# lukasc-ch/CBinfer

Measured on AMD Instinct MI355X. Metric: frames/sec + effective GFLOP/s vs dense, scene-labeling CNN 480x320 @10% change, higher is better.
Workload: dtype f32-equivalent: f32 tensors, every operand as three bf16 terms (24 bits, exact), six products on the bf16 MFMA, f32 accumulate; 1 GPU; sceneLabeling CBConv2d coarse-grained fp32, synthetic 480x320 seq @10% change (32x32 re-drawn blocks), experiment 6, one sequence per GPU; sequences_per_gpu=1, launch=program

## Files before the change

### cbinfer_amd/csrc/cb_split.hip

```cpp
#include <stdlib.h>

#include <type_traits>

#include "cb_common.h"

#ifdef CBS_STAMP
__device__ unsigned long long cbs_stamp_buf[4 * 2048 * 16];
#define CB_TAIL_STAMP(i)                                                                 \
    do {                                                                                 \
        if (threadIdx.x == 0 && blockIdx.x < 2048)                                       \
            cbs_stamp_buf[(2 * 2048 + blockIdx.x) * 16 + (i)] = __builtin_amdgcn_s_memrealtime(); \
    } while (0)
#define CBS_DET_STAMP(i)                                                                                            \
    do {                                                                                                            \
        const unsigned wg = blockIdx.y * gridDim.x + blockIdx.x;                                                    \
        if (POOL && threadIdx.x == 0 && blockIdx.z == 0 && wg < 2048)                                               \
            cbs_stamp_buf[(3 * 2048 + wg) * 16 + (i)] = __builtin_amdgcn_s_memrealtime();                            \
    } while (0)
#else
#define CBS_DET_STAMP(i)
#endif
#include "cb_tail_core.h"
#include "cb_split_common.h"

// ... 1468 lines not shown
                    }
                }
                __syncthreads();
#pragma unroll 1
                for (int c = 0; c < nNext; ++c) {
                    const CbhNext& nx = ext.L[q].next[c];
                    if (t < BN && ((s_nchg[c * (BN / 32) + (t >> 5)] >> (t & 31)) & 1u)) {
                        const int pix = s_tilePix[t];
                        const int py = cbs_div(pix, p.magicW), px = pix - py * p.W;
                        cbh_or_dilated(nx.masks, py, px, p.H, p.W, p.wpr, nx.kHH, nx.kWH);
                    }
                }
            }
        }
        CBS_STAMP_AT(5);
#ifdef CBS_STAMP
        cbs_first = false;
#endif
    }

    if constexpr (SIDE) {
        if (ext.sideFrame) {
            const int busy = min(items, (int)gridDim.x), nIdle = (int)gridDim.x - busy;
            const bool idleDo = nIdle >= 32;
            const int parts = idleDo ? nIdle : (int)gridDim.x, part = idleDo ? (int)blockIdx.x - busy : (int)blockIdx.x;
            if (part >= 0) {
                const int per = (ext.sideHW + parts - 1) / parts;
                const int i1 = min(ext.sideHW, (part + 1) * per);
                for (int i = part * per + t; i < i1; i += NT) {
                    bool chg = false;
                    for (int c = 0; c < ext.sideC; ++c)
                        chg |= cb_changed(ext.sideState[(long)c * ext.sideHW + i], ext.sideFrame[(long)c * ext.sideHW + i],
                                          ext.sideTh);
                    if (chg)
                        for (int c = 0; c < ext.sideC; ++c)
                            ext.sideState[(long)c * ext.sideHW + i] = ext.sideFrame[(long)c * ext.sideHW + i];
                }
            }
        }
    }

    if (totAll == 0) return;
    __syncthreads();
    if (t == 0) {
        int* ctl = (int*)(p.seq[0].masks + 2 * (long)MW);
        const int nSh = p.arriveShards;
        int last = 0;
        if (nSh <= 1) {
            last = __hip_atomic_fetch_add(ctl + 2, 1, __ATOMIC_RELAXED, __HIP_MEMORY_SCOPE_AGENT) == (int)gridDim.x - 1;
        } else {
            const int sh = blockIdx.x % nSh, expected = ((int)gridDim.x - sh + nSh - 1) / nSh;
            int* c = (int*)(p.seq[0].masks + (long)MW) + sh * 32;
            if (__hip_atomic_fetch_add(c, 1, __ATOMIC_RELAXED, __HIP_MEMORY_SCOPE_AGENT) == expected - 1) {
                __hip_atomic_store(c, 0, __ATOMIC_RELAXED, __HIP_MEMORY_SCOPE_AGENT);
                const int active = min(nSh, (int)gridDim.x);
                last = __hip_atomic_fetch_add(ctl + 2, 1, __ATOMIC_RELAXED, __HIP_MEMORY_SCOPE_AGENT) == active - 1;
            }
        }
        s_wsum[0] = last;
    }
    __syncthreads();
    if (s_wsum[0]) {
        for (int i = t; i < E; i += NT) {
            const int q = cbs_div(i, p.magicMW), w = i - q * MW;
            ((unsigned long long*)s_maskPtr[q])[w] = 0ull;
        }
        if (t == 0) {
            int* ctl = (int*)(p.seq[0].masks + 2 * (long)MW);
            __hip_atomic_store(ctl + 2, 0, __ATOMIC_RELAXED, __HIP_MEMORY_SCOPE_AGENT);
        }
    }
}

#define CBS_TILES_BEFORE(tilesBefore, info) \
    int tilesBefore[CBS_MAXSEQ + 1];        \
    tilesBefore[0] = 0;                     \
    _Pragma("unroll") for (int q_ = 0; q_ < CBS_MAXSEQ; ++q_) tilesBefore[q_ + 1] = tilesBefore[q_] + (info)[CBS_INFO_TP + q_]
#define CBS_TILE_SEQUENCE(q, tilesBefore, nSeq, ptg)  \
    int q = 0;                                        \
    _Pragma("unroll") for (int u_ = 1; u_ < CBS_MAXSEQ; ++u_) if (u_ < (nSeq) && (ptg) >= tilesBefore[u_]) q = u_

__global__ __launch_bounds__(256) void cbs_reduce_kernel(CbsParams p, int BM, int BN) {
    cb_touch_kernarg<sizeof(CbsParams) + 8>();
    const int SK = p.info[CBS_INFO_SK];
    if (SK <= 1) return;
    const int MT = p.info[CBS_INFO_MT], CMB = MT * SK, TILE4 = BM * BN / 4, HW = p.H * p.W;
    CBS_TILES_BEFORE(tilesBefore, p.info);
    const int TP = tilesBefore[CBS_MAXSEQ];
    const float4* __restrict__ slabs = (const float4*)p.slabs;
    const long total = (long)TP * MT * TILE4;
    for (long g = (long)blockIdx.x * 256 + threadIdx.x; g < total; g += (long)gridDim.x * 256) {
        const int tile = (int)(g / TILE4), c = (int)(g - (long)tile * TILE4);
        const int ptg = tile / MT, mt = tile % MT;
        const int nl = c % BN, mq = c / BN;
        CBS_TILE_SEQUENCE(q, tilesBefore, p.nSeq, ptg);
        const int n = (ptg - tilesBefore[q]) * BN + nl;
        const int N = p.info[CBS_INFO_TP + CBS_MAXSEQ + q];
        const float4* sl = slabs + ((long)ptg * CMB + mt) * TILE4 + c;
        const int pix = n < N ? p.seq[q].listOut[n] : -1;
        float s0 = 0.f, s1 = 0.f, s2 = 0.f, s3 = 0.f;
        for (int j0 = 0; j0 < SK; j0 += 8) {
            float4 v[8];
#pragma unroll
            for (int j = 0; j < 8; ++j)
                if (j0 + j < SK) v[j] = sl[(long)(j0 + j) * MT * TILE4];
#pragma unroll
            for (int j = 0; j < 8; ++j)
                if (j0 + j < SK) s0 += v[j].x, s1 += v[j].y, s2 += v[j].z, s3 += v[j].w;
        }
        if ((unsigned)pix >= (unsigned)HW) continue;
        const int m = mt * BM + 4 * mq;
        const float sv[4] = {s0, s1, s2, s3};
        float* out = p.seq[q].out;
#pragma unroll
        for (int e = 0; e < 4; ++e) {
            if (m + e >= p.K) continue;
            const float bv = !p.bias ? 0.f : (p.halfOut ? (float)((const _Float16*)p.bias)[m + e] : p.bias[m + e]);
            float v = fmaf(sv[e], p.outScale, bv);
            if (p.relu) v = v <= 0.f ? 0.f : v;
            if (p.halfOut) {
                ((_Float16*)out)[(long)(m + e) * HW + pix] = (_Float16)v;
                continue;
            }
            if (p.accumulate) {
                v += out[(long)(m + e) * HW + pix];
                float* rp = p.seq[q].reluOut;
                if (rp) rp[(long)(m + e) * HW + pix] = v <= 0.f ? 0.f : v;
            }
            out[(long)(m + e) * HW + pix] = v;
        }
    }
}

template <int BM, int BN>
__global__ __launch_bounds__(256) void cbh_reduce_kernel(CbsParams p, CbhExt ext) {
    cb_touch_kernarg<sizeof(CbsParams) + sizeof(CbhExt)>();
    if (p.info[CBS_INFO_SK] <= 1) return;
    const int MT = p.info[CBS_INFO_MT], TILE4 = BM * BN / 4, HW = p.H * p.W;
    int tilesBefore[CBH_GROUP + 1], slabBase[CBH_GROUP], chQ[CBH_GROUP];
    tilesBefore[0] = 0;
    {
        int run = 0;
#pragma unroll
        for (int q = 0; q < CBH_GROUP; ++q) {
            const int tq = p.info[CBS_INFO_TP + q];
            chQ[q] = p.info[CBS_INFO_CH + q];
            tilesBefore[q + 1] = tilesBefore[q] + tq;
            slabBase[q] = run;
            run += tq * MT * chQ[q];
        }
    }
    constexpr int PXG = 16, GP = BN / PXG;
    const int groups = tilesBefore[CBH_GROUP] * GP;
    const int t = threadIdx.x, px = t & 15;
    __shared__ unsigned s_chg[CBH_NEXT];
    const float4* __restrict__ slabs = (const float4*)p.slabs;
    const int QT = MT * (BM / 4);
    const int NCC = (QT + 31) / 32;
    for (int unit = blockIdx.x; unit < groups * NCC; unit += gridDim.x) {
        const int g = unit / NCC, cc = unit - g * NCC;
        const int ptg = g / GP, gi = g - ptg * GP;
        int q = 0;
#pragma unroll
        for (int u = 1; u < CBH_GROUP; ++u)
            if (u < p.nSeq && ptg >= tilesBefore[u]) q = u;
        const int n0 = (ptg - tilesBefore[q]) * BN + gi * PXG;
        const int N = p.info[CBS_INFO_TP + CBS_MAXSEQ + q];
        if (n0 >= N) continue;
        static_assert(CBH_GROUP == 2, "two layers");
        const int SK = q ? chQ[1] : chQ[0], CMB = MT * SK;
        const long tileSlab = (q ? slabBase[1] : slabBase[0]) + (long)(ptg - tilesBefore[q]) * CMB;
        const CbhLayer& L = ext.L[q];
        const int Kq = L.K, nNext = L.nNext;
        int pix = n0 + px < N ? p.seq[q].listOut[n0 + px] : -1;
        if ((unsigned)pix >= (unsigned)HW) pix = -1;
        const int pixLd = max(pix, 0);
        const int py = cbs_div(pixLd, p.magicW), pxx = pixLd - py * p.W;
        __syncthreads();
        if (t < CBH_NEXT) s_chg[t] = 0u;
        __syncthreads();
        _Float16* out = (_Float16*)p.seq[q].out;
        bool chg[CBH_NEXT];
#pragma unroll
        for (int c = 0; c < CBH_NEXT; ++c) chg[c] = false;
        const float4* sl0 = slabs + tileSlab * TILE4 + gi * PXG + px;
        const int nx2 = nNext > 1 ? 1 : 0;
        {
            const int cq0 = cc * 32 + (t >> 4);
            float4 v[2][8];
            _Float16 s4[2][CBH_NEXT][4];
            float acc[2][4];
#pragma unroll
            for (int u = 0; u < 2; ++u) {
                const int cq = min(cq0 + 16 * u, QT - 1);
                const int mt = cq / (BM / 4), mq = cq - mt * (BM / 4), m = mt * BM + 4 * mq;
                const float4* sl = sl0 + (long)mt * TILE4 + mq * BN;
#pragma unroll
                for (int j = 0; j < 8; ++j) v[u][j] = sl[(long)min(j, SK - 1) * MT * TILE4];
#pragma unroll
                for (int e = 0; e < 4; ++e) {
                    const long o = (long)min(m + e, Kq - 1) * HW + pixLd;
                    s4[u][0][e] = nNext > 0 ? L.next[0].state[o] : (_Float16)0;
                    if (CBH_NEXT > 1) s4[u][CBH_NEXT > 1 ? 1 : 0][e] = nNext > 0 ? L.next[nx2].state[o] : (_Float16)0;
                }
            }
#pragma unroll
            for (int u = 0; u < 2; ++u) {
                float s0 = 0.f, s1 = 0.f, s2 = 0.f, s3 = 0.f;
#pragma unroll
                for (int j = 0; j < 8; ++j)
                    if (j < SK) s0 += v[u][j].x, s1 += v[u][j].y, s2 += v[u][j].z, s3 += v[u][j].w;
                acc[u][0] = s0, acc[u][1] = s1, acc[u][2] = s2, acc[u][3] = s3;
            }
            if (SK > 8) {
#pragma unroll
                for (int u = 0; u < 2; ++u) {
                    const int cq = min(cq0 + 16 * u, QT - 1);
                    const int mt = cq / (BM / 4), mq = cq - mt * (BM / 4);
                    const float4* sl = sl0 + (long)mt * TILE4 + mq * BN;
#pragma unroll
                    for (int j = 0; j < 8; ++j) v[u][j] = sl[(long)min(8 + j, SK - 1) * MT * TILE4];
                }
#pragma unroll
                for (int u = 0; u < 2; ++u)
#pragma unroll
                    for (int j = 0; j < 8; ++j)
                        if (8 + j < SK)
                            acc[u][0] += v[u][j].x, acc[u][1] += v[u][j].y, acc[u][2] += v[u][j].z, acc[u][3] += v[u][j].w;
            }
#pragma unroll
            for (int u = 0; u < 2; ++u) {
                const int cq = cq0 + 16 * u;
                if (cq >= QT) continue;
                const int mt = cq / (BM / 4), mq = cq - mt * (BM / 4), m = mt * BM + 4 * mq;
                if (pix < 0 || m >= Kq) continue;
                _Float16 hv[4];
#pragma unroll
                for (int e = 0; e < 4; ++e) {
                    const float bv = (L.bias && m + e < Kq) ? (float)L.bias[m + e] : 0.f;
                    float r = fmaf(acc[u][e], p.outScale, bv);
                    if (L.relu) r = r <= 0.f ? 0.f : r;
                    hv[e] = m + e < Kq ? (_Float16)r : (_Float16)0;
                    if (m + e < Kq) out[(long)(m + e) * HW + pix] = hv[e];
                }
#pragma unroll
                for (int c = 0; c < CBH_NEXT; ++c) {
                    if (c >= nNext) continue;
                    const CbhNext& nx = L.next[c];
                    _Float16* nst = nx.state;
                    const _Float16 thc = (_Float16)nx.th;
                    unsigned dm = 0u;
                    bool ch = false;
#pragma unroll
                    for (int e = 0; e < 4; ++e) {
                        if (m + e >= Kq) continue;
                        ch |= cb_changed(s4[u][c][e], hv[e], thc);
                        dm |= (unsigned)cb_differs(s4[u][c][e], hv[e]) << e;
                    }
                    chg[c] |= ch;
                    if (dm) {
#pragma unroll
                        for (int e = 0; e < 4; ++e)
                            if ((dm >> e) & 1u) nst[(long)(m + e) * HW + pix] = hv[e];
                        if (m < (nx.rec >> 1)) {
                            typedef _Float16 halfx4 __attribute__((ext_vector_type(4)));
                            char* rec = nx.S + CBS_SPAD + ((long)(py + nx.padY) * nx.Wp + (pxx + nx.padXL)) * nx.rec;
                            *(halfx4*)(rec + m * 2) = halfx4{hv[0], hv[1], hv[2], hv[3]};
                        }
                    }
                }
            }
        }
        if (nNext > 0) {
#pragma unroll
            for (int c = 0; c < CBH_NEXT; ++c)
                if (c < nNext && chg[c]) atomicOr(&s_chg[c], 1u << px);
            __syncthreads();
            for (int c = 0; c < nNext; ++c) {
                const CbhNext& nx = L.next[c];
                const int dy = (t >> 4) - nx.kHH, yy = py + dy;
                if (pix >= 0 && ((s_chg[c] >> px) & 1u) && dy <= nx.kHH && yy >= 0 && yy < p.H)
                    cbh_or_dilated(nx.masks, yy, pxx, p.H, p.W, p.wpr, 0, nx.kWH);
            }
        }
    }
}

struct CbsTailArgs {
    const float* w1p;
    const float* b1;
    const float* w2;
    const float* b2;
    float* out[CBS_MAXSEQ];
    int C1, C2, relu1, relu2;
};
template <int BM, int BN, int S>
__global__ __launch_bounds__(S == 1 ? 64 * CB_TAIL_MAXW : CB_TAIL_MAXT) void cbs_reduce_tail_kernel(CbsParams p,
                                                                                                  CbsTailArgs ta) {
    extern __shared__ __attribute__((aligned(16))) float cbs_tail_sm[];
    cb_touch_kernarg<sizeof(CbsParams) + sizeof(CbsTailArgs)>();
    const int C0 = p.K, C0P = (C0 + 15) / 16 * 16, C1 = ta.C1, C2 = ta.C2, HW = p.H * p.W;
    const int t = threadIdx.x, NT = blockDim.x;
    CB_TAIL_STAMP(0);
    const int SK = p.info[CBS_INFO_SK], MT = p.info[CBS_INFO_MT], CMB = MT * SK, TILE4 = BM * BN / 4;
    CBS_TILES_BEFORE(tilesBefore, p.info);
    const int GP = BN / CB_TAIL_PX, groups = tilesBefore[CBS_MAXSEQ] * GP;
    if ((int)blockIdx.x >= groups) return;
    CB_TAIL_STAMP(1);
    const CbTailLds L = cb_tail_lds(cbs_tail_sm, C0P, C1, C2);
    __shared__ int s_pix[CB_TAIL_PX];
    for (int i = t; i < C2 * C1; i += NT) L.W2s[i] = ta.w2[i];
    for (int i = t; i < C2; i += NT) L.b2s[i] = ta.b2[i];
    const float4* __restrict__ slabs = (const float4*)p.slabs;
    const bool hasBias = p.bias != nullptr;
    const float* biasp = hasBias ? p.bias : ta.b1;
    const int px = t & 15, cstep = NT >> 4;
    for (int g = blockIdx.x; g < groups; g += gridDim.x) {
        const int ptg = g / GP, gi = g - ptg * GP;
        CBS_TILE_SEQUENCE(q, tilesBefore, p.nSeq, ptg);
        const int nl0 = gi * CB_TAIL_PX, n0 = (ptg - tilesBefore[q]) * BN + nl0;
        const int N = p.info[CBS_INFO_TP + CBS_MAXSEQ + q];
        if (n0 >= N) continue;
        float* outq = p.seq[q].out;
        float* relq = p.accumulate ? p.seq[q].reluOut : nullptr;
        int pixMine = -1;
        if (n0 + px < N) pixMine = p.seq[q].listOut[n0 + px];
        int tq = t >> 4;
        asm volatile("" : "+v"(tq));
        if ((unsigned)pixMine >= (unsigned)HW) pixMine = -1;
        const int pixLd = max(pixMine, 0);
        if (SK > 1) {
            const float4* sl0 = slabs + (long)ptg * CMB * TILE4 + nl0 + px;
            const int QN = C0P / 4, perThread = (QN + cstep - 1) / cstep;
            auto slabRounds = [&](auto uc) {
                constexpr int U = decltype(uc)::value;
                const int rounds = (QN + U * cstep - 1) / (U * cstep);
                for (int rd = 0; rd < rounds; ++rd) {
                    const int cq0 = tq + rd * U * cstep;
                    float4 v[U][CBS_CHUNKS], bq[U];
#pragma unroll
                    for (int u = 0; u < U; ++u) {
                        const int cq = min(cq0 + u * cstep, QN - 1), mt = cq / (BM / 4), mq = cq - mt * (BM / 4);
#pragma unroll
                        for (int j = 0; j < CBS_CHUNKS; ++j) v[u][j] = sl0[((long)j * MT + mt) * TILE4 + mq * BN];
                        bq[u] = *(const float4*)(biasp + (hasBias ? min(4 * cq, p.K - 4) : 0));
                    }
                    __builtin_amdgcn_sched_barrier(0);
                    if (rd == 0) {
                        __syncthreads();
                        if (t < CB_TAIL_PX) s_pix[t] = pixMine;
                        CB_TAIL_STAMP(2);
                    }
#pragma unroll
                    for (int u = 0; u < U; ++u) {
                        const int cq = cq0 + u * cstep;
                        float s0 = 0.f, s1 = 0.f, s2 = 0.f, s3 = 0.f;
#pragma unroll
                        for (int j = 0; j < CBS_CHUNKS; ++j)
                            s0 += v[u][j].x, s1 += v[u][j].y, s2 += v[u][j].z, s3 += v[u][j].w;
                        const float sv[4] = {s0, s1, s2, s3}, bv[4] = {bq[u].x, bq[u].y, bq[u].z, bq[u].w};
#pragma unroll
                        for (int e = 0; e < 4; ++e) {
                            const int m = 4 * cq + e;
                            float r = fmaf(sv[e], p.outScale, hasBias ? bv[e] : 0.f);
                            if (p.relu) r = r <= 0.f ? 0.f : r;
                            if (cq < QN) {
                                if (p.accumulate) {
                                    if (pixMine >= 0 && m < p.K) {
                                        r += outq[(long)m * HW + pixMine];
                                        outq[(long)m * HW + pixMine] = r;
                                        if (relq) {
                                            r = r <= 0.f ? 0.f : r;
                                            relq[(long)m * HW + pixMine] = r;
                                        }
                                    }
                                } else if (pixMine >= 0 && m < p.K) {
                                    outq[(long)m * HW + pixMine] = r;
                                }
                                L.Xs[m * CB_TAIL_PX + px] = (m < p.K && pixMine >= 0) ? r : 0.f;
                            }
                        }
                    }
                }
            };
            if (perThread <= 1) slabRounds(std::integral_constant<int, 1>());
            else if (perThread <= 2 || S > 1) slabRounds(std::integral_constant<int, 2>());
            else slabRounds(std::integral_constant<int, 4>());
        } else {
            __syncthreads();
            if (t < CB_TAIL_PX) s_pix[t] = pixMine;
            const float* gsrc = relq ? relq : outq;
            cb_tail_gather<(S == 1 ? 16 : 8)>(L.Xs, gsrc, HW, pixLd, pixMine >= 0, C0, C0P, tq, px, cstep);
        }
        asm volatile("" ::: "memory");
        CbTailPre<S> P;
        cb_tail_preload<S>(P, ta.w1p, ta.b1, C0P, C1);
        CB_TAIL_STAMP(3);
        cb_tail_tile<S>(L, s_pix, P, ta.w1p, ta.out[q], C0P, C1, C2, HW, ta.relu1, ta.relu2);
        CB_TAIL_STAMP(7);
    }
}

template <int BM, int BN, int WM, int WN, int PRE_CAP, bool MASK_LDS, int RING, int AR = 0>
int cbs_launch_conv(const CbsParams& p, int perCU, const CbsTailArgs* tail, hipStream_t s,
                    const typename CbsExtOf<AR>::type& ext = typename CbsExtOf<AR>::type()) {
    if ((long)p.nSeq * p.maskWords > PRE_CAP) return CB_ERR_UNSUPPORTED;
    const bool second = p.slabs && (p.nStages >= 48 || p.forceSK > 0);
    if (tail && !second) return CB_ERR_UNSUPPORTED;
    dim3 grid((unsigned)(perCU * cb_num_cus())), block(64 * WM * WN);
    hipLaunchKernelGGL((cbs_conv_kernel<BM, BN, WM, WN, PRE_CAP, MASK_LDS, RING, AR>), grid, block, 0, s, p, ext);
    int st = cb_launch_status();
    if (st != CB_OK) return st;
    if constexpr (AR == 1) {
        if (second) {
            hipLaunchKernelGGL((cbh_reduce_kernel<BM, BN>), dim3(2 * cb_num_cus()), dim3(256), 0, s, p, ext);
            st = cb_launch_status();
        }
        return st;
    }
    if (tail) {
        const int S = cb_tail_chain_sets(p.K, tail->C1);
        auto* k = S == 4 ? cbs_reduce_tail_kernel<BM, BN, 4> : S == 2 ? cbs_reduce_tail_kernel<BM, BN, 2>
                                                                      : cbs_reduce_tail_kernel<BM, BN, 1>;
        const int waves = (tail->C1 + 15) / 16 * S, perCU = waves > 8 ? 1 : 2;
        hipLaunchKernelGGL(k, dim3(perCU * cb_num_cus()), dim3(64 * waves), cb_tail_lds_bytes(p.K, tail->C1, tail->C2), s, p,
                           *tail);
        st = cb_launch_status();
    } else if (second) {
        hipLaunchKernelGGL(cbs_reduce_kernel, dim3(4 * cb_num_cus()), dim3(256), 0, s, p, BM, BN);
        st = cb_launch_status();
    }
    return st;
}

}
using namespace cbs;

#ifdef CBS_STAMP
extern "C" int cbinfer_debug_split_stamps(void* host, long bytes, int clear) {
    if (clear) {
        void* d = nullptr;
        if (hipGetSymbolAddress(&d, HIP_SYMBOL(cbs_stamp_buf)) != hipSuccess) return -1;
        return (int)hipMemset(d, 0, sizeof(unsigned long long) * 4 * 2048 * 16);
    }
    return (int)hipMemcpyFromSymbol(host, HIP_SYMBOL(cbs_stamp_buf), (size_t)bytes);
}
#endif

template <typename Ext>
static int cbs_fill_side(Ext& e, const cbSideRefresh* side) {
    CB_REQUIRE(side->state && side->C >= 1 && side->H >= 1 && side->W >= 1 && (long)side->H * side->W < (1l << 30));
    e.sideFrame = side->frame, e.sideState = side->state, e.sideC = side->C, e.sideHW = side->H * side->W;
    e.sideTh = side->threshold;
    return CB_OK;
}

extern "C" {

int cbinfer_split_supported(int C, int K, int kH, int kW) { return cbs_supported(C, K, kH, kW) ? 1 : 0; }
int cbinfer_split_max_sequences(void) { return CBS_MAXSEQ; }
long cbinfer_split_max_mask_words(int K) { return cbs_bm(K) >= 128 ? CBS_PRE_BIG : CBS_PRE_MID; }

long cbinfer_split_state_bytes(int C, int H, int W, int kH, int kW) {
    const CbsGeom g = cbs_geom(C, H, W, kH, kW);
    return CBS_SPAD + (long)g.Hp * g.Wp * g.rec;
}
long cbinfer_split3_state_bytes(int C, int H, int W, int kH, int kW) {
    const CbsGeom g = cbs_geom(C, H, W, kH, kW, 3);
    return CBS_SPAD + (long)g.Hp * g.Wp * g.rec;
}

static long cbs_plain_offset(long aBytes, int nStages) { return (aBytes + (long)nStages * 4 + 15) / 16 * 16; }
long cbinfer_split_prepared_bytes(int C, int K, int kH, int kW) {
    const CbsGeom g = cbs_geom(C, 64, 64, kH, kW);
    return cbs_plain_offset((long)g.nStages * (cbs_kp(K) / 32) * 4096, g.nStages) + (long)K * C * kH * kW * 4;
}
long cbinfer_split3_prepared_bytes(int C, int K, int kH, int kW) {
    const CbsGeom g = cbs_geom(C, 64, 64, kH, kW, 3);
    return cbs_plain_offset((long)g.nStages * (cbs_kp(K) / 32) * 6144, g.nStages);
}

static long cbs_slab_capacity(int nSeq, int H, int W, int K) {
    const int bm = cbs_bm(K), bn = bm >= 128 ? 128 : 64;
    const long tiles = (long)nSeq * (((long)H * W + bn - 1) / bn) * (cbs_kp(K) / bm);
    return tiles > 2l * cb_num_cus() ? tiles : 2l * cb_num_cus();
}
static long cbs_workspace_bytes(int nSeq, int H, int W, int K) {
    const int bm = cbs_bm(K), bn = bm >= 128 ? 128 : 64;
    return 256 + cbs_slab_capacity(nSeq, H, W, K) * bm * bn * 4;
}
long cbinfer_split_workspace_bytes(int nSeq, int C, int H, int W, int K, int kH, int kW) {
    if (!cbs_supported(C, K, kH, kW)) return 0;
    if (cbs_geom(C, H, W, kH, kW).nStages < 48) return 0;
    return cbs_workspace_bytes(nSeq, H, W, K);
}

static void cbs_fill_params(CbsParams& p, const CbsGeom& g, int K, int KP, int BM, int H, int W, long MW, void* workspace,
                            long cap) {
    p.info = workspace ? (int*)workspace : nullptr;
    p.slabs = workspace ? (float*)((char*)workspace + 256) : nullptr;
    p.K = K, p.KP = KP, p.H = H, p.W = W, p.Wp = g.Wp, p.rec = g.rec, p.nStages = g.nStages, p.kH = g.kH, p.kW = g.kW;
    p.maskWords = (int)MW, p.wpr = cbinfer_mask_words_per_row(W), p.dummyBase = g.dummyBase;
    p.stateBytes = (long)g.Hp * g.Wp * g.rec;
    p.magicMW = (1ull << 32) / (unsigned long long)MW + 1ull;
    p.magicWpr = (1ull << 32) / (unsigned long long)p.wpr + 1ull;
    p.magicW = (1ull << 32) / (unsigned long long)W + 1ull;
    p.magicMT = (1ull << 32) / (unsigned long long)(KP / BM) + 1ull;
    p.arriveShards = (int)(MW / 16 < 8 ? MW / 16 : 8);
    p.slabCap = (int)(cap > 0x7fffffffl ? 0x7fffffffl : cap);
    p.splitRounds = 2;
    p.dbg = 0;
}

static int cbs_prep_weights(const float* weight, void* prepared, int K, int C, int kH, int kW, int H, int W, int planes,
                            float weightScale, cbStream_t stream) {
    if (!cbs_supported(C, K, kH, kW)) return CB_ERR_UNSUPPORTED;
    const CbsGeom g = cbs_geom(C, H, W, kH, kW, planes);
    if ((long)g.Hp * g.Wp * g.rec >= (1l << 31)) return CB_ERR_UNSUPPORTED;
    const int KP = cbs_kp(K);
    const long total = (long)g.nStages * (KP / 32) * (2 * planes) * 64;
    const long aBytes = total * 16;
    int* stageOff = (int*)((char*)prepared + aBytes);
    float* wPlain = planes == 3 ? nullptr : (float*)((char*)prepared + cbs_plain_offset(aBytes, g.nStages));
    hipLaunchKernelGGL(cbs_prep_kernel, dim3(cb_div_up(total > g.nStages ? total : g.nStages, 256)), dim3(256), 0,
                       (hipStream_t)stream, weight, (halfx8*)prepared, stageOff, wPlain, g, K, KP, weightScale);
    return cb_launch_status();
}
int cbinfer_split_prep_weights(const float* weight, void* prepared, int K, int C, int kH, int kW, int H, int W,
                               float weightScale, cbStream_t stream) {
    CB_REQUIRE(weight && prepared && H > 0 && W > 0 && weightScale > 0.f);
    return cbs_prep_weights(weight, prepared, K, C, kH, kW, H, W, 2, weightScale, stream);
}
int cbinfer_split3_prep_weights(const float* weight, void* prepared, int K, int C, int kH, int kW, int H, int W,
                                cbStream_t stream) {
    CB_REQUIRE(weight && prepared && H > 0 && W > 0);
    return cbs_prep_weights(weight, prepared, K, C, kH, kW, H, W, 3, 1.0f, stream);
}

static int cbs_state_init(void* splitState, int C, int H, int W, int kH, int kW, int planes, cbStream_t stream) {
    CB_REQUIRE(splitState && H > 0 && W > 0);
    if (!cbs_supported(C, 1, kH, kW)) return CB_ERR_UNSUPPORTED;
    const CbsGeom g = cbs_geom(C, H, W, kH, kW, planes);
    hipLaunchKernelGGL(cbs_state_init_kernel, dim3(1024), dim3(256), 0, (hipStream_t)stream, (uint4*)splitState, g);
    return cb_launch_status();
}
int cbinfer_split_state_init(void* splitState, int C, int H, int W, int kH, int kW, cbStream_t stream) {
    return cbs_state_init(splitState, C, H, W, kH, kW, 2, stream);
}
int cbinfer_split3_state_init(void* splitState, int C, int H, int W, int kH, int kW, cbStream_t stream) {
    return cbs_state_init(splitState, C, H, W, kH, kW, 3, stream);
}

static int cbs_state_rebuild(const float* state, void* splitState, int C, int H, int W, int kH, int kW, int planes,
                             int32_t* rangeFlag, cbStream_t stream) {
    CB_REQUIRE(state && splitState && H > 0 && W > 0);
    if (!cbs_supported(C, 1, kH, kW)) return CB_ERR_UNSUPPORTED;
    const CbsGeom g = cbs_geom(C, H, W, kH, kW, planes);
    hipLaunchKernelGGL(cbs_state_rebuild_kernel, dim3(1024), dim3(256), 0, (hipStream_t)stream, state,
                       (char*)splitState, g, rangeFlag);
    return cb_launch_status();
}
int cbinfer_split_state_rebuild(const float* state, void* splitState, int C, int H, int W, int kH, int kW,
                                int32_t* rangeFlag, cbStream_t stream) {
    return cbs_state_rebuild(state, splitState, C, H, W, kH, kW, 2, rangeFlag, stream);
}
int cbinfer_split3_state_rebuild(const float* state, void* splitState, int C, int H, int W, int kH, int kW,
                                 cbStream_t stream) {
    return cbs_state_rebuild(state, splitState, C, H, W, kH, kW, 3, nullptr, stream);
}

int cbinfer_split_detect(const cbSplitSeq* seqs, int nSeq, int mode, int pH, int pW, int C, int H, int W,
                         int kH, int kW, float threshold, cbStream_t stream) {
    CB_REQUIRE(seqs && nSeq >= 1 && nSeq <= CBS_MAXSEQ && H > 0 && W > 0 && mode >= 0 && mode <= 15);
    const int x3 = (mode >> 3) & 1;
    const int pooled = mode & 1;
    const int fg = (mode >> 2) & 1;
    if (!cbs_supported(C, 1, kH, kW) || H > 65535) return CB_ERR_UNSUPPORTED;
    if (pooled) CB_REQUIRE((H == pH / 2 || H == (pH + 1) / 2) && (W == pW / 2 || W == (pW + 1) / 2));
    const CbsGeom g = cbs_geom(C, H, W, kH, kW, x3 ? 3 : 2);
    CbsDetArgs a;
    a.planes = g.planes;
    for (int q = 0; q < nSeq; ++q) {
        CB_REQUIRE(seqs[q].input && seqs[q].state && seqs[q].splitState && seqs[q].frameMasks);
        a.seq[q].in = seqs[q].input;
        a.seq[q].state = seqs[q].state;
        a.seq[q].S = (char*)seqs[q].splitState;
        a.seq[q].masks = (unsigned long long*)seqs[q].frameMasks;
        a.seq[q].prodMask = (pooled && !fg) ? (const unsigned long long*)seqs[q].producerMask : nullptr;
        a.seq[q].rangeFlag = x3 ? nullptr : seqs[q].rangeFlag;
        a.seq[q].delta = seqs[q].delta;
        if (fg) CB_REQUIRE(seqs[q].delta != nullptr);
    }
    a.W = W, a.H = H, a.C = C, a.kHH = (kH - 1) / 2, a.kWH = (kW - 1) / 2;
    a.wpr = cbinfer_mask_words_per_row(W), a.pH = pH, a.pW = pW;
    a.Wp = g.Wp, a.rec = g.rec, a.padY = g.padY, a.padXL = g.padXL;
    a.words = cbinfer_mask_words(H, W);
    a.th = threshold;
    a.copyAll = ((mode >> 1) & 1) | fg;
    a.fg = fg;
    dim3 grid(a.wpr, H, nSeq), block(64 * (C / 4));
    if (pooled)
        hipLaunchKernelGGL(cbs_detect_kernel<true>, grid, block, 0, (hipStream_t)stream, a);
    else
        hipLaunchKernelGGL(cbs_detect_kernel<false>, grid, block, 0, (hipStream_t)stream, a);
    return cb_launch_status();
}

static int cbs_detect_mode(int mode, float weightScale) {
    return (mode & ~CBINFER_SPLIT_X3) | (weightScale == 0.f ? CBINFER_SPLIT_X3 : 0);
}

static bool cbs_next_supported(int C, int K, int kH, int kW, int H, int W, const cbNextDetect* next) {
    if (!next || !cbs_supported(C, K, kH, kW) || K > 64 || K % 16 != 0 || !cbs_supported(K, 1, next->kH, next->kW)) return false;
    if (cbs_geom(C, H, W, kH, kW, 3).nStages >= 48) return false;
    if (!((next->H == H / 2 || next->H == (H + 1) / 2) && (next->W == W / 2 || next->W == (W + 1) / 2))) return false;
    if (next->arith != 0 && next->arith != 1) return false;
    const long MW = cbinfer_mask_words(H, W), EU = (long)((H + 1) / 2) * cbinfer_mask_words_per_row(W);
    if (MW > CBS_PRE_SMALL || 2 * EU + 2 > CBS_PRE_SMALL + 1 || EU + 1 > CBS_PRE_SMALL / 2 + 2) return false;
    const CbsGeom g2 = cbs_geom(K, next->H, next->W, next->kH, next->kW, next->arith ? 3 : 2);
    return (long)g2.Hp * g2.Wp * g2.rec < (1l << 31) && (long)H * W < (1l << 20);
}

static bool cbs_refresh_supported(int C, int K, int kH, int kW, int H, int W) {
    return cbs_supported(C, K, kH, kW) && K <= 64 && cbs_geom(C, H, W, kH, kW, 3).nStages < 48 &&
           cbinfer_mask_words(H, W) <= CBS_PRE_SMALL;
}

static int cbs_split_conv(const cbSplitSeq* seqs, int nSeq, const void* prepared, const float* bias, int C, int H,
                          int W, int K, int kH, int kW, float weightScale, int relu, void* workspace, int forceSplit,
                          const CbsTailArgs* tail, cbStream_t stream, int accumulate = 0,
                          const cbNextDetect* next = nullptr, const cbSideRefresh* side = nullptr) {
    if (workspace == nullptr && cbs_supported(C, K, kH, kW) && cbs_geom(C, H, W, kH, kW).nStages >= 48)
        return CB_ERR_BADARG;
    CB_REQUIRE(seqs && nSeq >= 1 && nSeq <= CBS_MAXSEQ && prepared && H > 0 && W > 0 && weightScale >= 0.f);
    if (!cbs_supported(C, K, kH, kW)) return CB_ERR_UNSUPPORTED;
    const bool x3 = weightScale == 0.f;
    const CbsGeom g = cbs_geom(C, H, W, kH, kW, x3 ? 3 : 2);
    const int KP = cbs_kp(K), BM = cbs_bm(K);
    const long MW = cbinfer_mask_words(H, W);
    if ((long)nSeq * MW > (BM >= 128 ? CBS_PRE_BIG : CBS_PRE_MID) || (long)g.Hp * g.Wp * g.rec >= (1l << 31) ||
        (long)H * W * W >= (1l << 32))
        return CB_ERR_UNSUPPORTED;
    CbsParams p;
    for (int q = 0; q < nSeq; ++q) {
        CB_REQUIRE(seqs[q].splitState && seqs[q].output && seqs[q].frameMasks && seqs[q].idxOut && seqs[q].countOut);
        p.seq[q].S = (const char*)seqs[q].splitState;
        p.seq[q].state = accumulate ? seqs[q].delta : seqs[q].state;
        p.seq[q].reluOut = accumulate ? seqs[q].reluOut : nullptr;
        p.seq[q].rangeFlag = (p.seq[q].state && !x3) ? seqs[q].rangeFlag : nullptr;
        p.seq[q].out = seqs[q].output;
        p.seq[q].masks = (unsigned long long*)seqs[q].frameMasks;
        p.seq[q].listOut = seqs[q].idxOut;
        p.seq[q].countOut = seqs[q].countOut;
        p.seq[q].maskCopy = (unsigned long long*)seqs[q].maskCopy;
    }
    p.nSeq = nSeq;
    p.aBytes = (long)g.nStages * (KP / 32) * (x3 ? 6144 : 4096);
    p.A = (const char*)prepared;
    p.stageOff = (const int*)((const char*)prepared + p.aBytes);
    p.wPlain = x3 ? nullptr : (const float*)((const char*)prepared + cbs_plain_offset(p.aBytes, g.nStages));
    p.bias = bias;
    p.relu = relu;
    cbs_fill_params(p, g, K, KP, BM, H, W, MW, workspace, cbs_slab_capacity(nSeq, H, W, K));
    p.outScale = x3 ? 1.0f : 1.0f / (weightScale * CBS_XSCALE);
    p.forceSK = forceSplit;
    p.accumulate = accumulate;
    p.halfOut = 0;
    p.upstream = nullptr;
    p.maxChunks = CBS_CHUNKS;
#ifdef CBS_DBG
    if (const char* e = getenv("CBINFER_SPLIT_DBG")) p.dbg = atoi(e);
#endif
    hipStream_t s = (hipStream_t)stream;
    if (side && side->frame && !next) {
        if (!cbs_refresh_supported(C, K, kH, kW, H, W) || nSeq != 1 || !x3 || accumulate || tail) return CB_ERR_UNSUPPORTED;
        CbsSideExt e;
        const int st = cbs_fill_side(e, side);
        if (st != CB_OK) return st;
        return cbs_launch_conv<64, 64, 2, 2, CBS_PRE_SMALL, true, 5, 4>(p, 1, nullptr, s, e);
    }
    if (next) {
        if (!cbs_next_supported(C, K, kH, kW, H, W, next) || nSeq != 1 || !x3 || accumulate || tail) return CB_ERR_UNSUPPORTED;
        CB_REQUIRE(next->state && next->splitState && next->frameMasks);
        const CbsGeom g2 = cbs_geom(K, next->H, next->W, next->kH, next->kW, next->arith ? 3 : 2);
        CbsWinExt e;
        e.nstate = next->state, e.nS = (char*)next->splitState, e.nmasks = (unsigned long long*)next->frameMasks;
        e.nflag = next->arith ? nullptr : next->rangeFlag;
        e.H2 = next->H, e.W2 = next->W, e.wpr2 = cbinfer_mask_words_per_row(next->W);
        e.kHH = (next->kH - 1) / 2, e.kWH = (next->kW - 1) / 2;
        e.Wp = g2.Wp, e.rec = g2.rec, e.padY = g2.padY, e.padXL = g2.padXL, e.planes = g2.planes;
        e.th = next->threshold;
        e.magicW2 = (1ull << 32) / (unsigned long long)next->W + 1ull;
        e.sideFrame = nullptr, e.sideState = nullptr, e.sideC = 0, e.sideHW = 0, e.sideTh = 0.f;
        if (side && side->frame) {
            const int st = cbs_fill_side(e, side);
            if (st != CB_OK) return st;
        }
        return cbs_launch_conv<64, 64, 2, 2, CBS_PRE_SMALL, true, 5, 3>(p, 1, nullptr, s, e);
    }
    if (x3) {
        if (BM == 128) {
            if ((long)nSeq * MW <= CBS_PRE_X3) return cbs_launch_conv<128, 128, 4, 2, CBS_PRE_X3, true, 3, 2>(p, 1, tail, s);
            return cbs_launch_conv<128, 128, 4, 2, CBS_PRE_BIG, false, 3, 2>(p, 1, tail, s);
// ... 522 lines not shown
```

Measured before the change: 11360 frames/s.

## Overlap tail kernel prologue loads with first slab burst via readlane info

Restructures the reduce-tail kernel prologue. Launch-info words now come in with one load per lane and are broadcast with readlane, replacing the scalar tilesBefore computation. W2/b2 weights are prefetched into registers and written to LDS only after the first group's slab loads are issued, and the listOut pixel index is loaded unconditionally so it overlaps with other loads. The goal is to hide global load latency at kernel start in a short-running tail kernel, at the cost of more register pressure and more intricate control flow, including explicit waitcnt calls.

```diff
diff --git a/cbinfer_amd/csrc/cb_split.hip b/cbinfer_amd/csrc/cb_split.hip
--- a/cbinfer_amd/csrc/cb_split.hip
+++ b/cbinfer_amd/csrc/cb_split.hip
@@ -1794,33 +1794,69 @@
     const int C0 = p.K, C0P = (C0 + 15) / 16 * 16, C1 = ta.C1, C2 = ta.C2, HW = p.H * p.W;
     const int t = threadIdx.x, NT = blockDim.x;
     CB_TAIL_STAMP(0);
-    const int SK = p.info[CBS_INFO_SK], MT = p.info[CBS_INFO_MT], CMB = MT * SK, TILE4 = BM * BN / 4;
-    CBS_TILES_BEFORE(tilesBefore, p.info);
-    const int GP = BN / CB_TAIL_PX, groups = tilesBefore[CBS_MAXSEQ] * GP;
+    constexpr int W2E = 2;
+    constexpr int NINFO = CBS_INFO_TP + 2 * CBS_MAXSEQ;
+    static_assert(NINFO <= 64, "a launch-info word per lane");
+    const int nW2 = C2 * C1;
+    const int iv = p.info[min(t & 63, NINFO - 1)];
+    float w2v[W2E];
+#pragma unroll
+    for (int e = 0; e < W2E; ++e) w2v[e] = ta.w2[min(t + e * NT, nW2 - 1)];
+    const float b2v = ta.b2[min(t, C2 - 1)];
+    __builtin_amdgcn_sched_barrier(0);
+    asm volatile("" ::: "memory");
+    const int SK = __builtin_amdgcn_readlane(iv, CBS_INFO_SK), MT = __builtin_amdgcn_readlane(iv, CBS_INFO_MT);
+    const int CMB = MT * SK, TILE4 = BM * BN / 4;
+    int tiles = 0;
+#pragma unroll
+    for (int q_ = 0; q_ < CBS_MAXSEQ; ++q_) tiles += __builtin_amdgcn_readlane(iv, CBS_INFO_TP + q_);
+    const int GP = BN / CB_TAIL_PX, groups = tiles * GP;
     if ((int)blockIdx.x >= groups) return;
     CB_TAIL_STAMP(1);
     const CbTailLds L = cb_tail_lds(cbs_tail_sm, C0P, C1, C2);
     __shared__ int s_pix[CB_TAIL_PX];
-    for (int i = t; i < C2 * C1; i += NT) L.W2s[i] = ta.w2[i];
-    for (int i = t; i < C2; i += NT) L.b2s[i] = ta.b2[i];
+    auto stageW2 = [&]() {
+#pragma unroll
+        for (int e = 0; e < W2E; ++e)
+            if (t + e * NT < nW2) L.W2s[t + e * NT] = w2v[e];
+        if (t < C2) L.b2s[t] = b2v;
+    };
+    auto stageW2Rest = [&]() {
+        for (int i = t + W2E * NT; i < nW2; i += NT) L.W2s[i] = ta.w2[i];
+        for (int i = t + NT; i < C2; i += NT) L.b2s[i] = ta.b2[i];
+    };
     const float4* __restrict__ slabs = (const float4*)p.slabs;
     const bool hasBias = p.bias != nullptr;
     const float* biasp = hasBias ? p.bias : ta.b1;
     const int px = t & 15, cstep = NT >> 4;
-    for (int g = blockIdx.x; g < groups; g += gridDim.x) {
-        const int ptg = g / GP, gi = g - ptg * GP;
-        CBS_TILE_SEQUENCE(q, tilesBefore, p.nSeq, ptg);
-        const int nl0 = gi * CB_TAIL_PX, n0 = (ptg - tilesBefore[q]) * BN + nl0;
-        const int N = p.info[CBS_INFO_TP + CBS_MAXSEQ + q];
-        if (n0 >= N) continue;
+    auto locate = [&](int g, int& ptg, int& q, int& nl0, int& n0, int& N) {
+        ptg = g / GP, nl0 = (g - ptg * GP) * CB_TAIL_PX;
+        int tilesBeforeQ = 0, before = 0;
+        q = 0, N = __builtin_amdgcn_readlane(iv, CBS_INFO_TP + CBS_MAXSEQ);
+#pragma unroll
+        for (int u = 1; u < CBS_MAXSEQ; ++u) {
+            before += __builtin_amdgcn_readlane(iv, CBS_INFO_TP + u - 1);
+            if (u < p.nSeq && ptg >= before)
+                q = u, tilesBeforeQ = before, N = __builtin_amdgcn_readlane(iv, CBS_INFO_TP + CBS_MAXSEQ + u);
+        }
+        n0 = (ptg - tilesBeforeQ) * BN + nl0;
+    };
+    auto group = [&](int g, auto firstc) {
+        constexpr bool FIRST = decltype(firstc)::value;
+        int ptg, q, nl0, n0, N;
+        locate(g, ptg, q, nl0, n0, N);
+        if constexpr (!FIRST)
+            if (n0 >= N) return;
         float* outq = p.seq[q].out;
         float* relq = p.accumulate ? p.seq[q].reluOut : nullptr;
-        int pixMine = -1;
-        if (n0 + px < N) pixMine = p.seq[q].listOut[n0 + px];
+        const int pixReq = p.seq[q].listOut[min(n0 + px, N - 1)];
         int tq = t >> 4;
         asm volatile("" : "+v"(tq));
-        if ((unsigned)pixMine >= (unsigned)HW) pixMine = -1;
-        const int pixLd = max(pixMine, 0);
+        auto pixOf = [&](int r) {
+            asm volatile("" : "+v"(r));
+            return (n0 + px < N && (unsigned)r < (unsigned)HW) ? r : -1;
+        };
+        int pixMine = -1;
         if (SK > 1) {
             const float4* sl0 = slabs + (long)ptg * CMB * TILE4 + nl0 + px;
             const int QN = C0P / 4, perThread = (QN + cstep - 1) / cstep;
@@ -1839,13 +1875,26 @@
                     }
                     __builtin_amdgcn_sched_barrier(0);
                     if (rd == 0) {
+                        if constexpr (FIRST) asm volatile("; cbs_tail_first_burst_end" ::: "memory");
+                        else asm volatile("; cbs_tail_next_burst_end" ::: "memory");
+                        __builtin_amdgcn_sched_barrier(0);
+                        pixMine = pixOf(pixReq);
+                        if constexpr (FIRST) stageW2();
                         __syncthreads();
                         if (t < CB_TAIL_PX) s_pix[t] = pixMine;
                         CB_TAIL_STAMP(2);
+#ifdef CBS_STAMP
+                        asm volatile("s_waitcnt vmcnt(0)" ::: "memory");
+                        CB_TAIL_STAMP(8);
+#endif
                     }
 #pragma unroll
                     for (int u = 0; u < U; ++u) {
                         const int cq = cq0 + u * cstep;
+#pragma unroll
+                        for (int j = 0; j < CBS_CHUNKS; ++j)
+                            asm volatile("" ::"v"(v[u][j].x), "v"(v[u][j].y), "v"(v[u][j].z), "v"(v[u][j].w));
+                        asm volatile("" ::"v"(bq[u].x), "v"(bq[u].y), "v"(bq[u].z), "v"(bq[u].w));
                         float s0 = 0.f, s1 = 0.f, s2 = 0.f, s3 = 0.f;
 #pragma unroll
                         for (int j = 0; j < CBS_CHUNKS; ++j)
@@ -1879,18 +1928,33 @@
             else if (perThread <= 2 || S > 1) slabRounds(std::integral_constant<int, 2>());
             else slabRounds(std::integral_constant<int, 4>());
         } else {
+            pixMine = pixOf(pixReq);
+            const int pixLd = max(pixMine, 0);
             __syncthreads();
             if (t < CB_TAIL_PX) s_pix[t] = pixMine;
             const float* gsrc = relq ? relq : outq;
             cb_tail_gather<(S == 1 ? 16 : 8)>(L.Xs, gsrc, HW, pixLd, pixMine >= 0, C0, C0P, tq, px, cstep);
-        }
+            __builtin_amdgcn_s_waitcnt(0x0f70);
+            if constexpr (FIRST) stageW2();
+        }
+        if constexpr (FIRST) stageW2Rest();
         asm volatile("" ::: "memory");
         CbTailPre<S> P;
         cb_tail_preload<S>(P, ta.w1p, ta.b1, C0P, C1);
         CB_TAIL_STAMP(3);
         cb_tail_tile<S>(L, s_pix, P, ta.w1p, ta.out[q], C0P, C1, C2, HW, ta.relu1, ta.relu2);
         CB_TAIL_STAMP(7);
-    }
+        if (g + (int)gridDim.x < groups) __builtin_amdgcn_s_waitcnt(0x0f70);
+    };
+    int g = blockIdx.x;
+    for (; g < groups; g += gridDim.x) {
+        int ptg, q, nl0, n0, N;
+        locate(g, ptg, q, nl0, n0, N);
+        if (n0 < N) break;
+    }
+    if (g >= groups) return;
+    group(g, std::true_type());
+    for (g += gridDim.x; g < groups; g += gridDim.x) group(g, std::false_type());
 }
 
 template <int BM, int BN, int WM, int WN, int PRE_CAP, bool MASK_LDS, int RING, int AR = 0>
```

After: 11510 frames/s (median of 6 runs). +1.3%, better.
